# architector1324/micro-raytracer

Measured on AMD Instinct MI355X. Metric: Msamples/sec (res x spp), higher is better.
Workload: dtype f32

## Files before the change

micro_raytracer_amd/csrc/mrt_api.cpp:

```cpp
#include <hip/hip_runtime_api.h>
#include <dlfcn.h>
#include <stdarg.h>
#include <stddef.h>
#include <stdio.h>
#include <stdlib.h>
#include <string.h>

#include <chrono>
#include <memory>
#include <mutex>
#include <string>
#include <utility>
#include <vector>

#include "../../include/mrt.h"
#include "mrt_denoise.h"
#include "mrt_kernels.h"
#include "mrt_pack.h"
#include "mrt_trace.h"

using namespace mrt;

namespace {

// ... 269 lines not shown
struct Plan {
    bool in_lds = true;
    u32 block_threads = 256;
    bool small_plain_grid = false;
    size_t staged_bytes = 0;
};

void plan_launch(const mrt_render_desc *desc, const mrt_desc_ext *ext, Packed &pk, Plan &pl)
{
    const bool no_lds = getenv("MRT_SCENE_IN_L2") != nullptr;
    const char *force = getenv("MRT_BLOCK_THREADS");
    const bool mesh_walk = pk.n_tbvh_nodes != 0u && (pk.features & 3u) == 3u;
    u32 deep_cap = kWalkCapDefault;
    if (const char *fw = getenv("MRT_WALK_CAP")) { const int v = atoi(fw); if (v >= 4 && v <= (int)kWalkCapMax) deep_cap = (u32)v; }
    pk.P.walk_cap = mesh_walk ? kLeafQueue : 0u;
    auto lds_of = [&](u32 shape, u32 marker) { return pt_lds_bytes(pk.P, shape, true, (pk.features & 31u) | marker); };
    auto fits = [&](u32 shape, u32 marker) { return lds_of(shape, marker) <= kLdsLimit; };
    auto fits_any = [&](u32 marker) { return fits(256u, marker) || fits(512u, marker) || fits(1024u, marker); };
    auto waves = [&](u32 shape, u32 marker) {
        const size_t l = lds_of(shape, marker);
        return l > kLdsLimit ? (size_t)0 : (shape / 64u) * (kLdsLimit / (l ? l : 1));
    };
    constexpr u32 kWarm = 64u, kDeep = 64u | 128u;
    const bool has_warm = pk.P.lds_words_warm < pk.P.lds_words || mesh_walk;
    u32 cold = 0u;
    bool in_lds = !no_lds;
    if (in_lds) {
        const char *fc = getenv("MRT_COLD");
        const char *fd = getenv("MRT_DEEP_NODES");
        const bool warm_ok = has_warm && fits_any(kWarm) && !(fc && !atoi(fc));
        const bool all_ok = fits_any(0u) && !(fc && atoi(fc) && warm_ok);
        const bool bvh_no_mesh = (pk.features & 16u) != 0u && (pk.features & 2u) == 0u;
        if (fd && mesh_walk) cold = kDeep;
        else if (mesh_walk && warm_ok && fits(1024u, kWarm)) cold = kWarm;
        else if (bvh_no_mesh && warm_ok && !fc && waves(256u, 0u) < 16u && waves(256u, kWarm) >= 24u) cold = kWarm;
        else if (all_ok) cold = 0u;
        else if (warm_ok) cold = kWarm;
        else if (mesh_walk) cold = kDeep;
        else in_lds = false;
        if (cold == kDeep) {
            PackOpts po; po.tbvh_wide = true;
            Packed again; std::string err2;
            bool ok2 = pack_scene(desc, again, err2, po, ext) == MRT_OK && again.tbvh_wide;
            const size_t fixed = (size_t)ST_SLOTS * 1024u * sizeof(float) + (size_t)deep_cap * 1024u * sizeof(u32) + 1024u;
            const size_t front = ok2 ? (size_t)again.P.off_tbvh * 4 : 0;
            ok2 = ok2 && front + fixed < kLdsLimit;
            if (ok2) {
                const size_t room = (kLdsLimit - fixed - front) / (B4_WORDS * 4);
                size_t n = fd ? (size_t)strtoul(fd, nullptr, 10) : room;
                if (n > room) n = room;
                if (n > again.n_tbvh_nodes) n = again.n_tbvh_nodes;
                const u32 n_mesh = (again.P.off_node - again.P.off_mesh) / MESH_WORDS;
                ok2 = n >= n_mesh && n_mesh > 0u;
                if (ok2) {
                    const u32 keep = pk.features;
                    pk = again;
                    pk.features = keep;
                    pk.P.walk_cap = deep_cap;
                    pk.P.n_tbvh_hot = (u32)n;
                    pk.P.lds_words_hot = (pk.P.off_tbvh + (u32)n * B4_WORDS + 3u) & ~3u;
                }
            }
            if (!ok2) { cold = 0u; in_lds = false; }
        }
    }
    const size_t full_bytes = (size_t)pk.P.lds_words * 4;
    const size_t blob_bytes = in_lds ? (size_t)staged_words_for(pk.P, cold) * 4 : full_bytes;
    u32 want = 256u, marker = cold;
    pl.small_plain_grid = false;
    if (in_lds) {
        const size_t w256 = waves(256u, cold), w512 = waves(512u, cold), w1024 = waves(1024u, cold);
        if (w256 >= 16u) { want = 256u; pl.small_plain_grid = blob_bytes <= kSmallScene && !cold; }
        else if (w512 >= 16u) want = 512u;
        else if (w1024 >= 16u) want = 1024u;
        else if (w256 >= w512 && w256 >= 8u) want = 256u;
        else if (!cold && fits(1024u, 32u)) { want = 1024u; marker |= 32u; }
        else want = w1024 ? 1024u : (w512 ? 512u : 256u);
    }
    if (force && in_lds) {
        const u32 f = (u32)atoi(force);
        if ((f == 64u && !cold) || f == 256u || f == 512u || f == 1024u) { if (fits(f, cold)) { want = f; marker = cold; pl.small_plain_grid = false; } }
    }
    pk.features = (pk.features & (31u | F_VATTR | F_ENV)) | marker | (pk.all_ident ? (u32)F_IDENT : 0u);
    if (in_lds && marker == kWarm && mesh_walk && has_walk_area(pk.features)) {
        const size_t w0 = waves(want, marker);
        while (pk.P.walk_cap < kWalkCapMax) {
            ++pk.P.walk_cap;
            if (waves(want, marker) != w0) { --pk.P.walk_cap; break; }
        }
    }
    pl.in_lds = in_lds;
    pl.block_threads = want;
    pl.staged_bytes = blob_bytes;
}

}

static mrt_ctx *create_single(const mrt_render_desc *desc, const mrt_opts *opts, const mrt_desc_ext *ext)
{
    const u32 shard_count = opts->shard_count ? opts->shard_count : 1;
    if (opts->shard_index >= shard_count) { fail(MRT_ERR_ARG, "mrt_create: shard_index %u >= shard_count %u", opts->shard_index, shard_count); return nullptr; }

    std::unique_ptr<mrt_ctx> c(new mrt_ctx());
    std::string err;
    const int rc = pack_scene(desc, c->pk, err, PackOpts(), ext);
    if (rc != MRT_OK) { fail(rc, "mrt_create: %s", err.c_str()); return nullptr; }
    Plan plan;
    plan_launch(desc, ext, c->pk, plan);
    if (c->pk.tbvh_wide) {
        c->aov_pk.reset(new Packed());
        if (pack_scene(desc, *c->aov_pk, err, PackOpts(), ext) != MRT_OK) { fail(MRT_ERR_SCENE, "mrt_create: %s", err.c_str()); return nullptr; }
    }

    int ndev = 0;
    if (hipGetDeviceCount(&ndev) != hipSuccess || ndev <= 0) { fail(MRT_ERR_DEVICE, "mrt_create: no HIP device (this backend has no CPU path)"); return nullptr; }
    int dev = opts->device;
    if (dev < 0) { if (hipGetDevice(&dev) != hipSuccess) dev = 0; }
    if (dev >= ndev) { fail(MRT_ERR_ARG, "mrt_create: device %d of %d", dev, ndev); return nullptr; }
    c->device = dev;
    c->seed = opts->seed;
    c->shard_index = opts->shard_index; c->shard_count = shard_count;
    c->shard_rows = opts->shard_rows ? opts->shard_rows : 8;

    const u32 nh = c->pk.nh;
    for (u32 y = 0; y < nh; ++y) if ((y / c->shard_rows) % shard_count == c->shard_index) c->row_of.push_back(y);
    c->local_rows = (u32)c->row_of.size();

    auto bail = [&](int code, const char *what, hipError_t e) { fail(code, "mrt_create: %s: %s", what, hipGetErrorString(e)); return (mrt_ctx *)nullptr; };
    hipError_t e;
    if ((e = hipSetDevice(dev)) != hipSuccess) return bail(MRT_ERR_DEVICE, "hipSetDevice", e);
    if ((e = create(c->stream)) != hipSuccess) return bail(MRT_ERR_DEVICE, "hipStreamCreate", e);
    if ((e = create(c->ev0)) != hipSuccess) return bail(MRT_ERR_DEVICE, "hipEventCreate", e);
    if ((e = create(c->ev1)) != hipSuccess) return bail(MRT_ERR_DEVICE, "hipEventCreate", e);
    const size_t all_words = c->pk.blob.size();
    if ((e = c->blob.alloc(all_words ? all_words : 4)) != hipSuccess) return bail(MRT_ERR_DEVICE, "hipMalloc(scene)", e);
    if ((e = hipMemcpy(c->blob.p, c->pk.blob.data(), all_words * 4, hipMemcpyHostToDevice)) != hipSuccess) return bail(MRT_ERR_DEVICE, "hipMemcpy(scene)", e);
    {
        const u32 n_blocks = (nh + c->shard_rows - 1) / c->shard_rows;
        c->padded_rows = ((n_blocks + shard_count - 1) / shard_count) * c->shard_rows;
        if (shard_count == 1) c->padded_rows = nh;
    }
    if ((e = c->accum_own.alloc(plane_floats(c.get()))) != hipSuccess) return bail(MRT_ERR_DEVICE, "hipMalloc(accumulator)", e);
    c->d_accum = c->accum_own.p;
    if ((e = hipMemset(c->d_accum, 0, plane_floats(c.get()) * sizeof(float))) != hipSuccess) return bail(MRT_ERR_DEVICE, "hipMemset", e);
    if ((e = c->segments.alloc(8)) != hipSuccess) return bail(MRT_ERR_DEVICE, "hipMalloc", e);
    if ((e = hipMemset(c->segments.p, 0, 8 * sizeof(unsigned long long))) != hipSuccess) return bail(MRT_ERR_DEVICE, "hipMemset", e);

    c->scene_in_lds = plan.in_lds;
    c->small_plain_grid = plan.small_plain_grid;
    const u32 want = plan.block_threads;
    const size_t blob_bytes = plan.staged_bytes;
    c->block_threads = want;
    c->pk.P.tiles_x = want == 64u ? 1u : (want == 256u ? 2u : 4u);
    c->pk.P.tiles_y = want == 64u ? 1u : (want == 1024u ? 4u : 2u);
    if (c->scene_in_lds && (e = configure_pt_once(dev)) != hipSuccess) return bail(MRT_ERR_DEVICE, "hipFuncSetAttribute", e);

    c->P = c->pk.P;
    c->P.local_rows = c->local_rows; c->P.shard_index = c->shard_index; c->P.shard_count = c->shard_count; c->P.shard_rows = c->shard_rows;
    c->P.seed_lo = (u32)c->seed; c->P.seed_hi = (u32)(c->seed >> 32);
    c->P.blob = c->blob.p; c->P.accum = c->d_accum; c->P.segments = c->segments.p;
    c->P.tile_counter = reinterpret_cast<u32 *>(c->segments.p + 1);
    {
        int n_cu = 0;
        if (!hip_tolerated(hipDeviceGetAttribute(&n_cu, hipDeviceAttributeMultiprocessorCount, c->device)) || n_cu <= 0) n_cu = 256;
        const size_t lds = pt_lds_bytes(c->pk.P, c->block_threads, c->scene_in_lds, c->pk.features);
        size_t per_cu = 32u / (c->block_threads / 64u);
// ... 1029 lines not shown
```

micro_raytracer_amd/csrc/mrt_pack.cpp:

```cpp
#include "mrt_pack.h"

#include <math.h>
#include <stdio.h>
#include <string.h>

#include <algorithm>
#include <map>
#include <array>

namespace mrt {
namespace {

constexpr u32 kBvhMinInstances = 24;

struct H3 { float x, y, z; };
inline H3 h3(float x, float y, float z) { H3 r = {x, y, z}; return r; }
inline H3 hadd(H3 a, H3 b) { return h3(a.x + b.x, a.y + b.y, a.z + b.z); }
inline H3 hsub(H3 a, H3 b) { return h3(a.x - b.x, a.y - b.y, a.z - b.z); }
inline H3 hmuls(H3 a, float s) { return h3(a.x * s, a.y * s, a.z * s); }
inline H3 hneg(H3 a) { return h3(-a.x, -a.y, -a.z); }
inline H3 hhadam(H3 a, H3 b) { return h3(a.x * b.x, a.y * b.y, a.z * b.z); }
inline float hdot(H3 a, H3 b) { return a.x * b.x + a.y * b.y + a.z * b.z; }
inline H3 hcross(H3 a, H3 b) { return h3(a.y * b.z - a.z * b.y, a.z * b.x - a.x * b.z, a.x * b.y - a.y * b.x); }
inline float hmag(H3 a) { return sqrtf(a.x * a.x + a.y * a.y + a.z * a.z); }
// ... 622 lines not shown
            instx_tab.insert(instx_tab.end(), ix, ix + INSTX_WORDS);
            Bound bd;
            bd.ok = o.kind != MRT_KIND_PLANE;
            for (int a = 0; a < 3; ++a) bd.mn[a] = bd.mx[a] = 0.0f;
            if (bd.ok) {
                double lo[3] = {0, 0, 0}, hi[3] = {0, 0, 0}, rad = 0.0;
                if (o.kind == MRT_KIND_SPHERE) { rad = fabs((double)o.param[0]); for (int a = 0; a < 3; ++a) { lo[a] = -rad; hi[a] = rad; } }
                else if (o.kind == MRT_KIND_BOX) {
                    rad = 0.5 * sqrt((double)o.param[0] * o.param[0] + (double)o.param[1] * o.param[1] + (double)o.param[2] * o.param[2]);
                    for (int a = 0; a < 3; ++a) { hi[a] = 0.5 * fabs((double)o.param[a]); lo[a] = -hi[a]; }
                } else {
                    const float *vs = o.kind == MRT_KIND_TRIANGLE ? o.param : o.tris;
                    const size_t nv = o.kind == MRT_KIND_TRIANGLE ? 3 : (size_t)o.n_tris * 3;
                    for (int a = 0; a < 3; ++a) { lo[a] = INFINITY; hi[a] = -INFINITY; }
                    for (size_t v = 0; v < nv; ++v) {
                        const float *q = vs + v * 3;
                        const double m = sqrt((double)q[0] * q[0] + (double)q[1] * q[1] + (double)q[2] * q[2]);
                        if (!(m <= rad)) rad = m;
                        for (int a = 0; a < 3; ++a) { if (!(q[a] >= lo[a])) lo[a] = q[a]; if (!(q[a] <= hi[a])) hi[a] = q[a]; }
                    }
                    if (nv == 0) for (int a = 0; a < 3; ++a) lo[a] = hi[a] = 0.0;
                }
                const float *X = xf_tab.data() + (size_t)xf * XF_WORDS;
                const bool ident = bits(X[XF_IDENT]) != 0;
                bool ortho = true;
                if (!ident) {
                    double M[9];
                    for (int a = 0; a < 3; ++a) for (int b2 = 0; b2 < 3; ++b2) { double acc = 0; for (int k = 0; k < 3; ++k) acc += (double)X[XF_R + a * 3 + k] * X[XF_L + k * 3 + b2]; M[a * 3 + b2] = acc; }
                    for (int a = 0; a < 3 && ortho; ++a) for (int b2 = 0; b2 < 3; ++b2) { double acc = 0; for (int k = 0; k < 3; ++k) acc += M[a * 3 + k] * M[b2 * 3 + k]; if (!(fabs(acc - (a == b2 ? 1.0 : 0.0)) < 1e-4)) ortho = false; }
                    for (int a = 0; a < 3; ++a) { lo[a] = -rad; hi[a] = rad; }
                }
                const double pp[3] = {pos.x, pos.y, pos.z};
                bd.ok = ortho && rad < 1e6;
                for (int a = 0; a < 3 && bd.ok; ++a) {
                    const double slack = 1e-3 * fmax(fabs(lo[a]), fabs(hi[a])) + 1e-6;
                    bd.mn[a] = (float)(pp[a] + lo[a] - slack); bd.mx[a] = (float)(pp[a] + hi[a] + slack);
                    if (!(fabs(pp[a]) < 1e6) || !(bd.mn[a] <= bd.mx[a])) bd.ok = false;
                }
            }
            bounds.push_back(bd);
        }
        n_inst_total += o.n_inst;

        u32 mr[MAT_WORDS] = {0};
        mr[MAT_ALBEDO] = bits(o.mat.albedo[0]); mr[MAT_ALBEDO + 1] = bits(o.mat.albedo[1]); mr[MAT_ALBEDO + 2] = bits(o.mat.albedo[2]);
        mr[MAT_ROUGH] = bits(o.mat.rough); mr[MAT_METAL] = bits(o.mat.metal); mr[MAT_GLASS] = bits(o.mat.glass);
        mr[MAT_OPACITY] = bits(o.mat.opacity); mr[MAT_EMIT] = bits(o.mat.emit);
        for (int k = 0; k < 6; ++k) mr[MAT_MAP + k] = (u32)maps[k];
        if (tex_bilinear && any_map) {
            mr[MAT_FLAGS] = MATF_BILINEAR | (o.kind == MRT_KIND_SPHERE ? (u32)MATF_CLAMP_V : 0u);
            out.features |= 512u | 1024u;
        }
        mat_tab.insert(mat_tab.end(), mr, mr + MAT_WORDS);
    }
    if (xf_tab.empty()) { const float dflt[4] = {-0.0f, -0.0f, -1.0f, -0.0f}; xf_of(dflt); }

    P.n_rend = sc.n_renderer; P.n_inst = n_inst_total; P.n_light = sc.n_light;
    if (sc.n_light) out.features |= 8u;
    P.off_rend = B.align4(); B.w.insert(B.w.end(), rend_tab.begin(), rend_tab.end());
    std::vector<u32> lin_list, bvh_inst;
    std::vector<float> bvh_nodes;
    {
        std::vector<u32> elig;
        for (u32 i = 0; i < n_inst_total; ++i) (bounds[i].ok ? elig : lin_list).push_back(i);
        if (n_inst_total < kBvhMinInstances || elig.size() < kBvhMinInstances / 2) {
            lin_list.clear(); elig.clear();
        } else {
            std::vector<TriBox> ib(n_inst_total);
            for (u32 i : elig) for (int a = 0; a < 3; ++a) { ib[i].mn[a] = bounds[i].mn[a]; ib[i].mx[a] = bounds[i].mx[a]; ib[i].c[a] = 0.5f * bounds[i].mn[a] + 0.5f * bounds[i].mx[a]; }
            TbvhBuild build{ib, bvh_nodes, bvh_inst, MRT_IBVH_LEAF_MAX};
            build.make(elig, 0, elig.size());
            const u32 n_nodes = (u32)(bvh_nodes.size() / BVH_WORDS);
            for (u32 k = 0; k < n_nodes; ++k) { float *q = bvh_nodes.data() + (size_t)k * BVH_WORDS; if (bits(q[BVH_SKIP]) >= n_nodes) q[BVH_SKIP] = fbits(BVH_END); }
            out.features |= 16u;
        }
    }
    P.n_lin = (u32)lin_list.size(); P.n_bvh_nodes = (u32)(bvh_nodes.size() / BVH_WORDS);
    out.all_ident = n_inst_total > 0;
    const u32 xf0 = n_inst_total ? inst_tab[INST_TAG] >> TAG_XF_SHIFT : 0u;
    for (u32 i = 0; i < n_inst_total && out.all_ident; ++i) {
        const u32 tag = inst_tab[(size_t)i * INST_WORDS + INST_TAG];
        out.all_ident = (tag & TAG_IDENT) != 0u && memcmp(&xf_tab[tag >> TAG_XF_SHIFT], &xf_tab[xf0], XF_IDENT * sizeof(float)) == 0;
    }
    {
        float r_min = 3.0e38f;
        bool sphere = false;
        for (u32 i : bvh_inst) {
            if ((inst_tab[(size_t)i * INST_WORDS + INST_TAG] & TAG_KIND_MASK) != KIND_SPHERE) continue;
            sphere = true;
            for (int a = 0; a < 3; ++a) r_min = std::min(r_min, 0.5f * (bounds[i].mx[a] - bounds[i].mn[a]));
        }
        P.inst_k = 1e-4f;
        P.inst_ksq = !sphere ? 0.0f : (r_min > 1e-12f ? 4e-6f / r_min : 1e30f);
        P.inst_kpos = sphere ? 1e-5f : 2e-6f;
    }
    out.n_lin = P.n_lin; out.n_bvh_nodes = P.n_bvh_nodes;
    P.off_cam = B.align4(); for (int k = 0; k < 9; ++k) B.f(P.cam_L[k]); for (int k = 0; k < 9; ++k) B.f(P.cam_R[k]);
    P.off_lin = B.align4(); B.w.insert(B.w.end(), lin_list.begin(), lin_list.end());
    P.off_bvh = B.align4(); for (float v : bvh_nodes) B.f(v);
    P.off_bvhinst = B.align4(); B.w.insert(B.w.end(), bvh_inst.begin(), bvh_inst.end());
    P.off_inst = B.align4(); B.w.insert(B.w.end(), inst_tab.begin(), inst_tab.end());
    P.off_instx = B.align4(); B.w.insert(B.w.end(), instx_tab.begin(), instx_tab.end());
    P.off_xf = B.align4(); for (float v : xf_tab) B.f(v);
    P.off_mat = B.align4(); B.w.insert(B.w.end(), mat_tab.begin(), mat_tab.end());
    P.off_light = B.align4();
    for (u32 l = 0; l < sc.n_light; ++l) {
        const mrt_light &li = sc.light[l];
        if (li.kind > MRT_LIGHT_DIR) { err = "unknown light kind"; return MRT_ERR_SCENE; }
        B.u(li.kind);
        if (li.kind == MRT_LIGHT_POINT) B.f3(h3(li.v[0], li.v[1], li.v[2]));
        else B.f3(hnorm(hneg(hnorm(h3(li.v[0], li.v[1], li.v[2])))));
        B.f(li.pwr);
        B.f3(h3(li.color[0], li.color[1], li.color[2]));
    }
    P.off_tex = B.align4();
    const u32 tex_desc0 = (u32)B.w.size();
    B.w.resize(B.w.size() + (size_t)sc.n_textures * TEX_WORDS, 0);
    P.off_lut = B.align4();
    for (int k = 0; k < 256; ++k) B.f((float)k / 255.0f);
    if (opts.tbvh_wide) {
        struct Ref { u32 depth, mesh, local; };
        std::vector<Ref> order;
        std::vector<std::vector<u32>> newi(wide.size());
        for (size_t m = 0; m < wide.size(); ++m) { newi[m].resize(wide[m].size()); for (size_t k = 0; k < wide[m].size(); ++k) order.push_back({wide[m][k].depth, (u32)m, (u32)k}); }
        std::stable_sort(order.begin(), order.end(), [](const Ref &a, const Ref &b) { return a.depth < b.depth; });
        if (order.size() >= (1u << 24)) { err = "triangle BVHs too large"; return MRT_ERR_LIMIT; }
        for (size_t k = 0; k < order.size(); ++k) newi[order[k].mesh][order[k].local] = (u32)k;
        tbvh_tab.assign(order.size() * B4_WORDS, 0.0f);
        for (size_t k = 0; k < order.size(); ++k) {
            const Wide4 &w = wide[order[k].mesh][order[k].local];
            float *q = tbvh_tab.data() + k * B4_WORDS;
            for (int c = 0; c < 4; ++c) {
                q[B4_CX + c] = w.c[c][0]; q[B4_CY + c] = w.c[c][1]; q[B4_CZ + c] = w.c[c][2];
                q[B4_HX + c] = w.h[c][0]; q[B4_HY + c] = w.h[c][1]; q[B4_HZ + c] = w.h[c][2];
                u32 cw = w.child[c];
                if (cw & B4_INTERNAL) cw = B4_INTERNAL | newi[order[k].mesh][cw & ~B4_INTERNAL];
                q[B4_CHILD + c] = fbits(cw);
            }
        }
        for (size_t m = 0; m < wide.size(); ++m) mesh_tab[(size_t)wide_mesh[m] * MESH_WORDS + MESH_TBVH] = newi[m][0];
        out.tbvh_wide = true;
    }
    P.off_mesh = B.align4(); B.w.insert(B.w.end(), mesh_tab.begin(), mesh_tab.end());
    P.off_node = B.align4(); for (float v : node_tab) B.f(v);
    P.off_parent = B.align4(); B.w.insert(B.w.end(), parent_tab.begin(), parent_tab.end());
    P.off_tbvh = B.align4(); for (float v : tbvh_tab) B.f(v);
    P.lds_words_hot = B.align4();
    P.off_tri = B.align4(); for (float v : tri_tab) B.f(v);
    P.off_memb = B.align4(); B.w.insert(B.w.end(), memb_tab.begin(), memb_tab.end());
    P.off_membe = B.align4(); B.w.insert(B.w.end(), membe_tab.begin(), membe_tab.end());
    P.lds_words_warm = B.align4();
    for (u32 t = 0; t < sc.n_textures; ++t) {
        const mrt_texture &tx = sc.textures[t];
        u32 *desc = B.w.data() + tex_desc0 + (size_t)t * TEX_WORDS;
        desc[TEX_W] = tx.w; desc[TEX_H] = tx.h;
        if (!tx.dat) { desc[TEX_FMT] = TEXFMT_NONE; continue; }
        const size_t n = (size_t)tx.w * tx.h * 3;
        bool exact = true;
        for (size_t i = 0; i < n && exact; ++i) {
            const float v = tx.dat[i];
            const float kf = rintf(v * 255.0f);
            exact = kf >= 0.0f && kf <= 255.0f && bits(kf / 255.0f) == bits(v);
        }
        const u32 off = B.align4();
        desc = B.w.data() + tex_desc0 + (size_t)t * TEX_WORDS;
        if (exact) {
            desc[TEX_FMT] = TEXFMT_U8; desc[TEX_OFF] = off * 4u;
            std::vector<unsigned char> bytes(n);
            for (size_t i = 0; i < n; ++i) bytes[i] = (unsigned char)rintf(tx.dat[i] * 255.0f);
            const size_t words = (n + 3) / 4;
            const size_t at = B.w.size();
            B.w.resize(at + words, 0);
            memcpy(B.w.data() + at, bytes.data(), n);
            out.n_tex_u8++;
        } else {
            desc[TEX_FMT] = TEXFMT_F32; desc[TEX_OFF] = off;
            for (size_t i = 0; i < n; ++i) B.f(tx.dat[i]);
            out.n_tex_f32++;
        }
    }
    P.off_leaf = B.align4(); B.w.insert(B.w.end(), leaf_tab.begin(), leaf_tab.end());
    P.lds_words = P.off_leaf;
    if (!vattr_tab.empty()) {
        out.off_vattr = B.align4(); for (float v : vattr_tab) B.f(v);
        out.n_vattr_rows = (u32)(vattr_tab.size() / VATTR_WORDS);
// ... 39 lines not shown
```

micro_raytracer_amd/csrc/mrt_pack.h:

```cpp
#pragma once
#include <string>
#include <vector>

#include "../../include/mrt.h"
#include "mrt_scene.h"

namespace mrt {

struct Packed {
    Params P;
    std::vector<u32> blob;
    u32 nw = 0, nh = 0;
    u32 res_w = 0, res_h = 0;
    float gamma = 0, exp = 0;
    u32 features = 0;
    bool all_ident = false;
    bool tbvh_wide = false;
    u32 n_tex_u8 = 0, n_tex_f32 = 0, n_nodes = 0, n_leaf_ids = 0, n_tris = 0, n_xf = 0, n_bvh_nodes = 0, n_lin = 0, n_tbvh_nodes = 0;
    u32 off_vattr = 0, n_vattr_rows = 0;
};

struct PackOpts {
    bool tbvh_wide = false;
};

int pack_scene(const mrt_render_desc *desc, Packed &out, std::string &err, const PackOpts &opts = PackOpts(), const mrt_desc_ext *ext = nullptr);

struct OctreeFlat {
    std::vector<float> nodes;
    std::vector<u32> leaf_ids;
    u32 root = NO_NODE;
    bool empty_root = false;
};
void build_octree(const float *tris, u32 n_tris, OctreeFlat &out);

bool build_tbvh(const float *tris, u32 n_tris, std::vector<float> &nodes, std::vector<u32> &order);

struct ResampleTaps {
    std::vector<u32> left;
    std::vector<u32> count;
    std::vector<float> weight;
    u32 cap = 0;
};
void lanczos3_taps(u32 src, u32 dst, ResampleTaps &out);

}
```

micro_raytracer_amd/csrc/mrt_scene.h:

```cpp
#pragma once
#include <stddef.h>

#include "mrt_math.h"

namespace mrt {

constexpr u32 REND_WORDS = 16;
constexpr u32 INST_WORDS = 8;
constexpr u32 XF_WORDS = 20;
constexpr u32 MAT_WORDS = 16;
constexpr u32 LIGHT_WORDS = 8;
constexpr u32 TEX_WORDS = 4;
constexpr u32 MESH_WORDS = 12;
constexpr u32 TRI_WORDS = 9;
constexpr u32 NODE_WORDS = 8;

enum : u32 { REND_KIND = 0, REND_INST_OFF = 1, REND_INST_CNT = 2, REND_FLAGS = 3, REND_GEO = 4 };
enum : u32 { RF_HAS_MAPS = 1u, RF_HAS_UV = 2u, RF_HAS_VN = 4u };
enum : u32 { REND_VATTR = 15 };
constexpr u32 VATTR_WORDS = 16;
enum : u32 { VATTR_VN = 0, VATTR_UV = 9 };

enum : u32 { INST_POS = 0, INST_P3 = 3, INST_TAG = 4, INST_P5 = 5 };
enum : u32 { INSTX_REND = 0, INSTX_PLANE_NW = 1 };
constexpr u32 INSTX_WORDS = 4;
constexpr u32 TAG_KIND_MASK = 7u, TAG_IDENT = 8u, TAG_XF_SHIFT = 4u;

enum : u32 { XF_L = 0, XF_R = 9, XF_IDENT = 18 };

enum : u32 { MAT_ALBEDO = 0, MAT_ROUGH = 3, MAT_METAL = 4, MAT_GLASS = 5, MAT_OPACITY = 6, MAT_EMIT = 7, MAT_MAP = 8, MAT_FLAGS = 14 };
enum : u32 { MATF_BILINEAR = 1u, MATF_CLAMP_V = 2u };
enum : u32 { MAP_TEX = 0, MAP_ROUGH = 1, MAP_METAL = 2, MAP_GLASS = 3, MAP_OPACITY = 4, MAP_EMIT = 5 };

enum : u32 { LIGHT_KIND = 0, LIGHT_V = 1, LIGHT_PWR = 4, LIGHT_COLOR = 5 };

enum : u32 { TEX_W = 0, TEX_H = 1, TEX_OFF = 2, TEX_FMT = 3 };
enum : u32 { TEXFMT_NONE = 0, TEXFMT_F32 = 1, TEXFMT_U8 = 2 };

enum : u32 { ENV_W = 0, ENV_H = 1, ENV_OFF = 2, ENV_FMT = 3, ENV_MAP = 4, ENV_ROT = 5, ENV_PWR = 6, ENV_FLAGS = 7 };
enum : u32 { ENVF_BILINEAR = 1u };
constexpr u32 ENV_WORDS = 8;
enum : u32 { ENVMAP_SPHERE = 0, ENVMAP_LATLONG = 1 };

enum : u32 { MESH_TRI0 = 0, MESH_NTRI = 1, MESH_ROOT = 2, MESH_LEAF0 = 3, MESH_TBVH = 4, MESH_NIDS = 5, MESH_BC = 6, MESH_BH = 9 };
constexpr u32 NO_NODE = 0xffffffffu;

enum : u32 { NODE_HALF = 0, NODE_REL = 3, NODE_FIRST = 6, NODE_COUNT = 7 };

constexpr u32 B4_WORDS = 28;
constexpr u32 B4_INTERNAL = 0x80000000u;
constexpr u32 kWalkCapMin = 8u, kWalkCapMax = 16u, kWalkCapDefault = 16u;
enum : u32 { B4_CX = 0, B4_CY = 4, B4_CZ = 8, B4_HX = 12, B4_HY = 16, B4_HZ = 20, B4_CHILD = 24 };
constexpr u32 BVH_WORDS = 8;
constexpr u32 MEMB_SLOT_BITS = 22u, MEMB_SLOT_MASK = (1u << MEMB_SLOT_BITS) - 1u;
enum : u32 { BVH_C = 0, BVH_H = 3, BVH_SKIP = 6, BVH_LEAF = 7 };
constexpr u32 BVH_END = 0xffffffffu;

enum : u32 { KIND_SPHERE = 0, KIND_PLANE = 1, KIND_BOX = 2, KIND_TRIANGLE = 3, KIND_MESH = 4 };
enum : u32 { LK_POINT = 0, LK_DIR = 1 };

constexpr u32 kChunk = 16;

struct Params {
    u32 nw, nh;
    u32 local_rows, shard_index, shard_count, shard_rows;
    u32 n_samples, sample_base;
    u32 k_split;
    u32 to_planes;
    u32 seed_lo, seed_hi;
    u32 bounce;
    float q;
    float w, h, aspect;
    float inv2tan;
    float cam_pos[3];
    float aprt, foc;
    float cam_L[9], cam_R[9];
    u32 cam_ident;
    float sky[3];
    float sky_init[3];
    u32 n_rend, n_light, n_inst;
    u32 n_lin, n_bvh_nodes;
    float inst_ksq;
    float inst_k, inst_kpos;
    u32 off_lin, off_bvh, off_bvhinst;
    u32 off_cam;
    u32 off_rend, off_inst, off_instx, off_xf, off_mat, off_light, off_tex, off_lut, off_mesh, off_tri, off_node, off_leaf;
    u32 off_tbvh, off_memb, off_membe, off_parent;
    u32 n_tbvh_hot;
    u32 walk_cap;
    u32 blob_words;
    u32 lds_words;
    u32 lds_words_warm;
    u32 lds_words_hot;
    u32 tiles_x, tiles_y;
    u32 count_segments;
    const u32 *blob;
    float *accum;
    float *partial;
    unsigned long long partial_stride;
    unsigned long long *segments;
    u32 *tile_counter;
    u32 persist_grid;
    u32 off_env;
};
static_assert(sizeof(Params) % 8 == 0 && offsetof(Params, off_env) + 4 == sizeof(Params), "off_env fills the tail of Params");

struct TileList {
    const u32 *tiles;
    u32 n;
};

}
```

micro_raytracer_amd/csrc/mrt_trace.h:

```cpp
#pragma once
#include "mrt_scene.h"

namespace mrt {

enum : u32 {
    F_BOX = 1u,
    F_TRI = 2u,
    F_MAPS = 4u,
    F_LIGHTS = 8u,
    F_ALL = 15u,
    F_BVH = 16u,
    F_NOSTASH = 32u,
    F_COLD = 64u,
    F_DEEP = 128u,
    F_IDENT = 256u,
    F_ENV = 1024u,
    F_VATTR = 512u
};
constexpr u32 plain_feat(u32 feat) { return feat & ~(u32)F_IDENT; }
MRT_HD u32 staged_words_for(const Params &P, u32 feat) { return (feat & F_DEEP) ? P.lds_words_hot : ((feat & F_COLD) ? P.lds_words_warm : P.lds_words); }
constexpr bool has_walk_area(u32 feat) { return (feat & F_TRI) && (feat & F_BOX) && (feat & F_COLD); }
#ifndef MRT_UNIFORM_TAG
#define MRT_UNIFORM_TAG 1
#endif
#ifndef MRT_T0_FROM_KEY
#define MRT_T0_FROM_KEY 1
#endif
#ifndef MRT_NZFIN_PRODUCT
#define MRT_NZFIN_PRODUCT 1
#endif
#ifndef MRT_SHADOW_QUEUE
#define MRT_SHADOW_QUEUE 0
#endif
#ifndef MRT_LEAF_QUEUE
#define MRT_LEAF_QUEUE 8u
#endif
constexpr u32 kLeafQueue = MRT_LEAF_QUEUE;

#ifndef MRT_PROBE
#define MRT_PROBE(phase)
#endif
#ifndef MRT_COUNT
#define MRT_COUNT(counter)
#endif
#ifndef MRT_PROBE_INST
#define MRT_PROBE_INST(i)
#endif
#if defined(MRT_PHASE_TIMING) && defined(__HIP_DEVICE_COMPILE__)
#define MRT_TICK(slot) do { const unsigned long long now_ = __builtin_amdgcn_s_memtime(); phase_ticks[slot] += now_ - phase_last; phase_last = now_; } while (0)
#define MRT_TICK_DECL unsigned long long phase_ticks[4] = {0ull, 0ull, 0ull, 0ull}; unsigned long long phase_last = __builtin_amdgcn_s_memtime()
#define MRT_TICK_OUT(dst) do { for (int k_ = 0; k_ < 4; ++k_) (dst)[k_] = phase_ticks[k_]; } while (0)
#else
#define MRT_TICK(slot)
#define MRT_TICK_DECL
#define MRT_TICK_OUT(dst)
#endif
#ifndef MRT_PROBE_FALLBACK
#define MRT_PROBE_FALLBACK(ro, rd, dd)
#endif
#ifndef MRT_PROBE_ROUND
#define MRT_PROBE_ROUND(steps, tris, membs)
#endif
enum : u32 { CT_TRACE = 0, CT_LIN_TEST, CT_BVH_NODE, CT_BVH_TEST, CT_MESH_CALL, CT_MESH_ROOT_HIT, CT_TBVH_NODE, CT_TBVH_TRI, CT_TBVH_TRI_HIT, CT_MEMB_BOX, CT_TRACE_ANY, CT_WALK_OVERFLOW, CT_WALK_ROUND, CT_REF_TRI, CT_REF_BOX, CT_COUNT };
enum : u32 { PH_ITER = 0, PH_REGEN, PH_SPHERE_MATH, PH_PLANE_HIT, PH_SHADE, PH_NORMAL_NONPLANE, PH_SCATTER1, PH_SCATTER2, PH_REFRACT, PH_EMIT_END, PH_LIGHTS, PH_COUNT };

constexpr float kE = 0.0001f;
constexpr float kBig = 1.0f / 0.0001f;

struct V3 { float x, y, z; };
MRT_HD V3 v3(float x, float y, float z) { V3 r; r.x = x; r.y = y; r.z = z; return r; }
MRT_HD V3 add(V3 a, V3 b) { return v3(a.x + b.x, a.y + b.y, a.z + b.z); }
MRT_HD V3 sub(V3 a, V3 b) { return v3(a.x - b.x, a.y - b.y, a.z - b.z); }
MRT_HD float dot(V3 a, V3 b) { return a.x * b.x + a.y * b.y + a.z * b.z; }
MRT_HD V3 muls(V3 a, float s) { return v3(a.x * s, a.y * s, a.z * s); }
MRT_HD V3 neg(V3 a) { return v3(-a.x, -a.y, -a.z); }
MRT_HD V3 hadam(V3 a, V3 b) { return v3(a.x * b.x, a.y * b.y, a.z * b.z); }
MRT_HD V3 cross(V3 a, V3 b) { return v3(a.y * b.z - a.z * b.y, a.z * b.x - a.x * b.z, a.x * b.y - a.y * b.x); }
MRT_HD float mag(V3 a) { return sqrt_(a.x * a.x + a.y * a.y + a.z * a.z); }
MRT_HD V3 norm(V3 a) { return muls(a, recip_sqrt_(a.x * a.x + a.y * a.y + a.z * a.z)); }
MRT_HD V3 reflect(V3 d, V3 n) { return sub(d, muls(n, 2.0f * dot(d, n))); }
MRT_HD V3 m3mul(const float *m, V3 v)
{
    return v3(m[0] * v.x + m[1] * v.y + m[2] * v.z, m[3] * v.x + m[4] * v.y + m[5] * v.z, m[6] * v.x + m[7] * v.y + m[8] * v.z);
}
MRT_HD V3 ld3(const float *F, u32 i) { return v3(F[i], F[i + 1], F[i + 2]); }
struct alignas(16) F4 { float x, y, z, w; };
MRT_HD F4 ld4(const float *F, u32 i) { return *reinterpret_cast<const F4 *>(F + i); }
MRT_HD u32 ldu(const float *F, u32 i) { return f2u(F[i]); }

MRT_HD bool nzfin(float x)
{
#if defined(__HIP_DEVICE_COMPILE__)
    return __builtin_amdgcn_classf(x, 0x198);
#else
    const float a = fabs_(x);
    return a > 0.0f && a < kInf;
#endif
}
MRT_HD bool nzfin3(V3 v) { return nzfin(v.x) && nzfin(v.y) && nzfin(v.z); }
MRT_HD bool nzfin3_product(V3 v) { return MRT_NZFIN_PRODUCT ? nzfin((v.x * v.y) * v.z) : nzfin3(v); }
MRT_HD u32 mul24(u32 a, u32 b)
{
    return (a & 0xffffffu) * (b & 0xffffffu);
}
MRT_HD void sched_fence()
{
#if defined(__HIP_DEVICE_COMPILE__)
    __builtin_amdgcn_sched_barrier(0);
#endif
}
MRT_HD u32 opaque_v(u32 x)
{
#if defined(__HIP_DEVICE_COMPILE__)
    asm volatile("" : "+v"(x));
#endif
    return x;
}
MRT_HD u32 opaque_s(u32 x)
{
#if defined(__HIP_DEVICE_COMPILE__)
    asm volatile("" : "+s"(x));
#endif
    return x;
}
MRT_HD u32 lowest_bit(u32 x) { return (u32)__builtin_ctz(x | 0x80000000u); }

MRT_HD V3 xf_full(const float *X, V3 v) { return m3mul(X + XF_R, m3mul(X + XF_L, v)); }
MRT_HD V3 xf_vec(const float *X, bool ident, V3 v)
{
    if (ident && nzfin3_product(v)) return v;
    return xf_full(X, v);
}

MRT_HD V3 recip_patched(V3 d)
{
    V3 m;
#if defined(MRT_FAST_IEEE)
    if (wave_all(in_window(d.x) && in_window(d.y) && in_window(d.z))) {
        m = v3(div_core_(1.0f, d.x, rcp_refined_(d.x)), div_core_(1.0f, d.y, rcp_refined_(d.y)), div_core_(1.0f, d.z, rcp_refined_(d.z)));
        return m;
    }
#endif
    m = v3(1.0f / d.x, 1.0f / d.y, 1.0f / d.z);
    if (fabs_(m.x) == kInf) m.x = kBig;
    if (fabs_(m.y) == kInf) m.y = kBig;
    if (fabs_(m.z) == kInf) m.z = kBig;
    return m;
}

MRT_HD bool box_isect(V3 half, V3 ro, V3 m, V3 pos, float &t0, float &t1)
{
    const V3 n = hadam(sub(ro, pos), m);
    const V3 k = hadam(half, v3(fabs_(m.x), fabs_(m.y), fabs_(m.z)));
    const V3 a = sub(neg(n), k);
    const V3 b = add(neg(n), k);
    t0 = fmax_(fmax_(a.x, a.y), a.z);
    t1 = fmin_(fmin_(b.x, b.y), b.z);
    return !(t0 > t1 || t1 < 0.0f);
}

MRT_HD bool sphere_isect(float r2, V3 oo, V3 rd, float a, float &t0, float &t1)
{
    const float b = 2.0f * dot(oo, rd);
    const float c = dot(oo, oo) - r2;
    const float disc = b * b - 4.0f * a * c;
    if (disc < 0.0f) return false;
    if (b > 1e-20f && a > 0.0f && a < 1e18f && disc >= 0.0f) return false;
    MRT_PROBE(PH_SPHERE_MATH);
    const float sq = sqrt_(disc);
    float q0, q1;
    div2_(-b - sq, -b + sq, 2.0f * a, q0, q1);
// ... 689 lines not shown
template <bool ANY, u32 FEAT, bool UNIFORM = false>
MRT_HD bool isect_instance(const Scn &S, const RayPre &ray, u32 i, const F4 &ia, const F4 &ib, float &t0, float &t1, i32 &i0, i32 &i1, const float *X0 = nullptr)
{
    const float *F = S.U;
    const Params &P = *S.P;
    const V3 pos = v3(ia.x, ia.y, ia.z);
    const u32 tag = (UNIFORM && (FEAT & F_TRI) && MRT_UNIFORM_TAG) ? wave_uniform(f2u(ib.x)) : f2u(ib.x);
    const u32 kind = (UNIFORM && (FEAT & F_IDENT)) ? wave_uniform(tag & TAG_KIND_MASK) : (tag & TAG_KIND_MASK);
    const bool ident = (FEAT & F_IDENT) ? true : (tag & TAG_IDENT) != 0;
    const float *X = (FEAT & F_IDENT) ? X0 : F + P.off_xf + (tag >> TAG_XF_SHIFT);
    const V3 ro = add(pos, xf_vec(X, ident, sub(ray.o, pos)));
    const bool fast_d = (FEAT & F_IDENT) ? true : (ident && ray.d_ok);
    V3 rd = ray.d, m = ray.m;
    float dd = ray.dd;
    if (!fast_d) {
        rd = xf_full(X, ray.d);
        if constexpr (FEAT & F_BOX) m = recip_patched(rd);
        dd = dot(rd, rd);
    }
    t0 = 0.0f; t1 = 0.0f; i0 = -1; i1 = -1;
    if (kind == KIND_SPHERE) return sphere_isect(ia.w, sub(ro, pos), rd, dd, t0, t1);
    if (kind == KIND_PLANE) { const bool h = plane_isect(v3(ib.y, ib.z, ib.w), ia.w, ro, rd, t0); t1 = t0; return h; }
    if ((FEAT & F_BOX) && kind == KIND_BOX) return box_isect(v3(ia.w, ib.y, ib.z), ro, m, pos, t0, t1);
    if (FEAT & F_TRI) {
        const float *R = F + P.off_rend + ldu(F, P.off_instx + i * INSTX_WORDS + INSTX_REND) * REND_WORDS;
        if (kind == KIND_TRIANGLE) {
            const bool h = tri_isect(add(ld3(R, REND_GEO), pos), ld3(R, REND_GEO + 3), ld3(R, REND_GEO + 6), ro, rd, t0);
            t1 = t0;
            return h;
        }
        if ((FEAT & F_BOX) && kind == KIND_MESH) return mesh_isect<ANY, FEAT>(S, ldu(R, REND_GEO), ro, rd, dd, m, pos, t0, i0, t1, i1);
    }
    return false;
}

template <bool V> struct BoolTag { static constexpr bool value = V; };

template <bool ANY, u32 FEAT>
MRT_HD bool trace(const Scn &S, const RayPre &ray_, Hit &best)
{
    const float *F = S.U;
    const Params &P = *S.P;
    i32 best_key = 0x7fffffff;
    best.rend = -1; best.inst = 0; best.t0 = 0.0f; best.t1 = 0.0f; best.i0 = -1; best.i1 = -1;
    const float *I = F + P.off_inst;

    if (ANY) { MRT_COUNT(CT_TRACE_ANY); } else { MRT_COUNT(CT_TRACE); }
    const float *X0 = nullptr;
    RayPre ray_i = ray_;
    if constexpr (FEAT & F_IDENT) {
        X0 = F + P.off_xf + (ldu(I, INST_TAG) >> TAG_XF_SHIFT);
        if (!ray_.d_ok) {
            ray_i.d = xf_full(X0, ray_.d);
            if constexpr (FEAT & F_BOX) ray_i.m = recip_patched(ray_i.d);
            ray_i.dd = dot(ray_i.d, ray_i.d);
        }
    }
    const RayPre &ray = ray_i;
    auto consider = [&](u32 i, const F4 &ia, const F4 &ib, auto in_order, auto uniform) -> bool {
        float t0, t1;
        MRT_COUNT(CT_LIN_TEST);
        MRT_PROBE_INST(i);
        i32 i0, i1;
        if (!isect_instance<ANY, FEAT, decltype(uniform)::value>(S, ray, i, ia, ib, t0, t1, i0, i1, X0)) return false;
        if (ANY) return true;
        const i32 key = total_key(t0);
        const unsigned long long pair = ((unsigned long long)((u32)key ^ 0x80000000u) << 32) | i;
        const unsigned long long best_pair = ((unsigned long long)((u32)best_key ^ 0x80000000u) << 32) | (best.rend < 0 ? 0xffffffffu : best.inst);
        const bool better = decltype(in_order)::value ? key < best_key : pair < best_pair;
        if (better) {
            best_key = key;
            best.rend = 0; best.inst = i; best.t1 = t1; best.i0 = i0; best.i1 = i1;
            if constexpr ((FEAT & F_BVH) != 0 || !MRT_T0_FROM_KEY) best.t0 = t0;
        }
        return false;
    };
    using InOrder = BoolTag<(FEAT & F_BVH) == 0>;
    using AnyOrder = BoolTag<false>;
    using Shared = BoolTag<true>;
    using PerLane = BoolTag<false>;

    const bool bvh = (FEAT & F_BVH) != 0;
    const u32 n = bvh ? P.n_lin : P.n_inst;
    if (!bvh && !(FEAT & F_TRI) && n) {
        u32 j = 0;
        F4 a0 = ld4(I, 0), a1 = ld4(I, 4), b0 = a0, b1 = a1;
        for (;;) {
            if (j + 1u < n) { b0 = ld4(I, (j + 1u) * INST_WORDS); b1 = ld4(I, (j + 1u) * INST_WORDS + 4); }
            if (consider(j, a0, a1, InOrder(), Shared())) return true;
            if (++j >= n) break;
            if (j + 1u < n) { a0 = ld4(I, (j + 1u) * INST_WORDS); a1 = ld4(I, (j + 1u) * INST_WORDS + 4); }
            if (consider(j, b0, b1, InOrder(), Shared())) return true;
            if (++j >= n) break;
        }
    } else if (n) {
        const float *Lst = F + P.off_lin;
        u32 cur = bvh ? ldu(Lst, 0) : 0u;
        F4 qa = ld4(I, cur * INST_WORDS), qb = ld4(I, cur * INST_WORDS + 4);
        for (u32 j = 0; j < n; ++j) {
            const F4 ia = qa, ib = qb;
            const u32 i = cur;
            if (j + 1 < n) {
                cur = bvh ? ldu(Lst, j + 1) : j + 1;
                qa = ld4(I, cur * INST_WORDS); qb = ld4(I, cur * INST_WORDS + 4);
            }
            if (consider(i, ia, ib, InOrder(), Shared())) return true;
        }
    }

    if constexpr (bvh) {
        const bool cull = cull_ok(ray_.o, ray_.dd);
        const CullRay R = cull_ray(ray_.o, ray_.d);
        const float *N0 = F + P.off_bvh;
        u32 node = P.n_bvh_nodes ? 0u : BVH_END;
        V3 oinv, qm;
        float mg;
        {
            const F4 ra = ld4(N0, 0), rb = ld4(N0, 4);
            const V3 r = sub(v3(ra.x, ra.y, ra.z), R.o);
            const float ext = fmax_(fmax_(fabs_(r.x) + ra.w, fabs_(r.y) + rb.x), fabs_(r.z) + rb.y);
            const float obig = fmax_(fmax_(fabs_(ray_.o.x), fabs_(ray_.o.y)), fabs_(ray_.o.z));
            const float ksq = fmin_(P.inst_ksq * ext, 4e-3f) * MRT_MARGIN_SCALE;
            mg = fma_fast(P.inst_k * MRT_MARGIN_SCALE + ksq, ext, fma_fast(P.inst_kpos * MRT_MARGIN_SCALE, obig + obig + ext, 1e-6f * MRT_MARGIN_SCALE));
            oinv = hadam(R.o, R.inv);
            qm = muls(R.ainv, mg);
        }
        for (;;) {
            u32 leaf_a = 0u, leaf_b = 0u;
            bool walking = node != BVH_END;
            const float far = (!ANY && best.rend >= 0 && best.t0 >= 0.0f) ? best.t0 + 1e-3f * best.t0 + mg : kInf;
            while (walking) {
                const F4 na = ld4(N0, node * BVH_WORDS), nb = ld4(N0, node * BVH_WORDS + 4);
                MRT_COUNT(CT_BVH_NODE);
                const u32 skip = f2u(nb.z), leaf = f2u(nb.w);
                const float px = fma_fast(na.x, R.inv.x, -oinv.x), py = fma_fast(na.y, R.inv.y, -oinv.y), pz = fma_fast(na.z, R.inv.z, -oinv.z);
                const float qx = fma_fast(na.w, R.ainv.x, qm.x), qy = fma_fast(nb.x, R.ainv.y, qm.y), qz = fma_fast(nb.y, R.ainv.z, qm.z);
                const float tn = fmax_(fmax_(px - qx, py - qy), pz - qz);
                const float tf = fmin_(fmin_(px + qx, py + qy), pz + qz);
                bool hit_node = !(tn > tf || tf < 0.0f);
                if (!ANY) hit_node = hit_node && !(tn > far);
                hit_node = hit_node || !cull;
                const u32 cand = hit_node ? leaf : 0u;
                const bool have_a = leaf_a != 0u;
                leaf_b |= have_a ? cand : 0u;
                leaf_a |= have_a ? 0u : cand;
                node = (hit_node && leaf == 0u) ? node + 1u : skip;
                walking = node != BVH_END && leaf_b == 0u;
            }
            if (leaf_a == 0u) break;
            const u32 cnt_a = leaf_a >> 24, first_a = leaf_a & 0xffffffu, cnt_b = leaf_b >> 24, first_b = leaf_b & 0xffffffu;
            for (u32 k = 0; k < cnt_a + cnt_b; ++k) {
                const u32 i = ldu(F, P.off_bvhinst + (k < cnt_a ? first_a + k : first_b + (k - cnt_a)));
                if (consider(i, ld4(I, i * INST_WORDS), ld4(I, i * INST_WORDS + 4), AnyOrder(), PerLane())) return true;
            }
        }
    }
    if (best.rend < 0) return false;
    if constexpr ((FEAT & F_BVH) == 0 && MRT_T0_FROM_KEY) {
        const i32 k = best_key;
        best.t0 = u2f((u32)(k ^ (i32)(((u32)(k >> 31)) >> 1)));
    }
    best.rend = (i32)ldu(S.F, P.off_instx + best.inst * INSTX_WORDS + INSTX_REND);
    return true;
}

struct Obj {
    const float *R, *IX, *X;
// ... 469 lines not shown
```

Baseline: 9292.

## Add axis-aligned plane fast scan for identity-transform sphere/plane scenes

At pack time, scenes whose instances all share an identity transform and contain only spheres and axis-aligned planes get a compact per-instance table holding the plane axis code and signed distance. The trace loop gains a specialised linear scan for that case. It intersects axis-aligned planes with a single division along one axis instead of the general plane test, and keeps the sphere test. The aim is to cut arithmetic and instance-record loads in the primary intersection loop. The cost is extra code paths, a wave-uniform branch on the axis code, and float-exactness assumptions checked through bounds and wave_all guards. An env var can disable it.

```diff
diff --git a/micro_raytracer_amd/csrc/mrt_api.cpp b/micro_raytracer_amd/csrc/mrt_api.cpp
--- a/micro_raytracer_amd/csrc/mrt_api.cpp
+++ b/micro_raytracer_amd/csrc/mrt_api.cpp
@@ -375,6 +375,7 @@
         if ((f == 64u && !cold) || f == 256u || f == 512u || f == 1024u) { if (fits(f, cold)) { want = f; marker = cold; pl.small_plain_grid = false; } }
     }
     pk.features = (pk.features & (31u | F_VATTR | F_ENV)) | marker | (pk.all_ident ? (u32)F_IDENT : 0u);
+    if (const char *fa = getenv("MRT_AXIS_SCAN")) { if (!atoi(fa)) pk.P.axis_scan = 0u; }
     if (in_lds && marker == kWarm && mesh_walk && has_walk_area(pk.features)) {
         const size_t w0 = waves(want, marker);
         while (pk.P.walk_cap < kWalkCapMax) {
diff --git a/micro_raytracer_amd/csrc/mrt_pack.cpp b/micro_raytracer_amd/csrc/mrt_pack.cpp
--- a/micro_raytracer_amd/csrc/mrt_pack.cpp
+++ b/micro_raytracer_amd/csrc/mrt_pack.cpp
@@ -728,6 +728,26 @@
         const u32 tag = inst_tab[(size_t)i * INST_WORDS + INST_TAG];
         out.all_ident = (tag & TAG_IDENT) != 0u && memcmp(&xf_tab[tag >> TAG_XF_SHIFT], &xf_tab[xf0], XF_IDENT * sizeof(float)) == 0;
     }
+    std::vector<u32> axis_tab;
+    out.axis_scan = out.all_ident && out.features == 0u;
+    for (u32 i = 0; i < n_inst_total && out.axis_scan; ++i) {
+        const u32 *ir = &inst_tab[(size_t)i * INST_WORDS];
+        const u32 kind = ir[INST_TAG] & TAG_KIND_MASK;
+        auto bounded = [](u32 w) { return fabsf(fbits(w)) <= kAxisMax; };
+        u32 code = 0u, sd = 0u;
+        bool ok = bounded(ir[INST_POS]) && bounded(ir[INST_POS + 1]) && bounded(ir[INST_POS + 2]) && bounded(ir[INST_P3]);
+        if (kind == KIND_PLANE) {
+            u32 ones = 0u, zeros = 0u;
+            for (u32 k = 0; k < 3u; ++k) {
+                const u32 w = ir[INST_P5 + k], mag = w & 0x7fffffffu;
+                if (mag == 0x3f800000u) { ++ones; code = k + 1u; sd = ir[INST_P3] ^ (w & 0x80000000u); }
+                else if (mag == 0u) ++zeros;
+            }
+            ok = ok && ones == 1u && zeros == 2u;
+        } else if (kind != KIND_SPHERE) ok = false;
+        axis_tab.push_back(code); axis_tab.push_back(sd);
+        out.axis_scan = ok;
+    }
     {
         float r_min = 3.0e38f;
         bool sphere = false;
@@ -747,6 +767,8 @@
     P.off_bvhinst = B.align4(); B.w.insert(B.w.end(), bvh_inst.begin(), bvh_inst.end());
     P.off_inst = B.align4(); B.w.insert(B.w.end(), inst_tab.begin(), inst_tab.end());
     P.off_instx = B.align4(); B.w.insert(B.w.end(), instx_tab.begin(), instx_tab.end());
+    P.off_axis = 0u; P.axis_scan = out.axis_scan ? 1u : 0u;
+    if (out.axis_scan) { P.off_axis = B.align4(); B.w.insert(B.w.end(), axis_tab.begin(), axis_tab.end()); }
     P.off_xf = B.align4(); for (float v : xf_tab) B.f(v);
     P.off_mat = B.align4(); B.w.insert(B.w.end(), mat_tab.begin(), mat_tab.end());
     P.off_light = B.align4();
diff --git a/micro_raytracer_amd/csrc/mrt_pack.h b/micro_raytracer_amd/csrc/mrt_pack.h
--- a/micro_raytracer_amd/csrc/mrt_pack.h
+++ b/micro_raytracer_amd/csrc/mrt_pack.h
@@ -15,6 +15,7 @@
     float gamma = 0, exp = 0;
     u32 features = 0;
     bool all_ident = false;
+    bool axis_scan = false;
     bool tbvh_wide = false;
     u32 n_tex_u8 = 0, n_tex_f32 = 0, n_nodes = 0, n_leaf_ids = 0, n_tris = 0, n_xf = 0, n_bvh_nodes = 0, n_lin = 0, n_tbvh_nodes = 0;
     u32 off_vattr = 0, n_vattr_rows = 0;
diff --git a/micro_raytracer_amd/csrc/mrt_scene.h b/micro_raytracer_amd/csrc/mrt_scene.h
--- a/micro_raytracer_amd/csrc/mrt_scene.h
+++ b/micro_raytracer_amd/csrc/mrt_scene.h
@@ -24,6 +24,9 @@
 enum : u32 { INST_POS = 0, INST_P3 = 3, INST_TAG = 4, INST_P5 = 5 };
 enum : u32 { INSTX_REND = 0, INSTX_PLANE_NW = 1 };
 constexpr u32 INSTX_WORDS = 4;
+enum : u32 { AXIS_CODE = 0, AXIS_SD = 1 };
+constexpr u32 AXIS_WORDS = 2;
+constexpr float kAxisMax = 0x1p38f;
 constexpr u32 TAG_KIND_MASK = 7u, TAG_IDENT = 8u, TAG_XF_SHIFT = 4u;
 
 enum : u32 { XF_L = 0, XF_R = 9, XF_IDENT = 18 };
@@ -102,8 +105,10 @@
     u32 *tile_counter;
     u32 persist_grid;
     u32 off_env;
+    u32 off_axis;
+    u32 axis_scan;
 };
-static_assert(sizeof(Params) % 8 == 0 && offsetof(Params, off_env) + 4 == sizeof(Params), "off_env fills the tail of Params");
+static_assert(sizeof(Params) % 8 == 0 && offsetof(Params, axis_scan) + 4 == sizeof(Params), "Params has no tail padding");
 
 struct TileList {
     const u32 *tiles;
diff --git a/micro_raytracer_amd/csrc/mrt_trace.h b/micro_raytracer_amd/csrc/mrt_trace.h
--- a/micro_raytracer_amd/csrc/mrt_trace.h
+++ b/micro_raytracer_amd/csrc/mrt_trace.h
@@ -61,7 +61,7 @@
 #ifndef MRT_PROBE_ROUND
 #define MRT_PROBE_ROUND(steps, tris, membs)
 #endif
-enum : u32 { CT_TRACE = 0, CT_LIN_TEST, CT_BVH_NODE, CT_BVH_TEST, CT_MESH_CALL, CT_MESH_ROOT_HIT, CT_TBVH_NODE, CT_TBVH_TRI, CT_TBVH_TRI_HIT, CT_MEMB_BOX, CT_TRACE_ANY, CT_WALK_OVERFLOW, CT_WALK_ROUND, CT_REF_TRI, CT_REF_BOX, CT_COUNT };
+enum : u32 { CT_TRACE = 0, CT_LIN_TEST, CT_BVH_NODE, CT_BVH_TEST, CT_MESH_CALL, CT_MESH_ROOT_HIT, CT_TBVH_NODE, CT_TBVH_TRI, CT_TBVH_TRI_HIT, CT_MEMB_BOX, CT_TRACE_ANY, CT_WALK_OVERFLOW, CT_WALK_ROUND, CT_REF_TRI, CT_REF_BOX, CT_AXIS_SCAN, CT_COUNT };
 enum : u32 { PH_ITER = 0, PH_REGEN, PH_SPHERE_MATH, PH_PLANE_HIT, PH_SHADE, PH_NORMAL_NONPLANE, PH_SCATTER1, PH_SCATTER2, PH_REFRACT, PH_EMIT_END, PH_LIGHTS, PH_COUNT };
 
 constexpr float kE = 0.0001f;
@@ -87,6 +87,8 @@
 struct alignas(16) F4 { float x, y, z, w; };
 MRT_HD F4 ld4(const float *F, u32 i) { return *reinterpret_cast<const F4 *>(F + i); }
 MRT_HD u32 ldu(const float *F, u32 i) { return f2u(F[i]); }
+struct alignas(8) F2 { float x, y; };
+MRT_HD F2 ld2(const float *F, u32 i) { return *reinterpret_cast<const F2 *>(F + i); }
 
 MRT_HD bool nzfin(float x)
 {
@@ -942,7 +944,66 @@
 
     const bool bvh = (FEAT & F_BVH) != 0;
     const u32 n = bvh ? P.n_lin : P.n_inst;
-    if (!bvh && !(FEAT & F_TRI) && n) {
+    bool scanned = false;
+    if constexpr (!ANY && FEAT == F_IDENT && MRT_T0_FROM_KEY) {
+        const V3 o = ray_.o, d = ray_.d;
+        const bool tame = (int)in_window(d.x) & (int)in_window(d.y) & (int)in_window(d.z) & (int)(fabs_(o.x) <= kAxisMax) & (int)(fabs_(o.y) <= kAxisMax) &
+                          (int)(fabs_(o.z) <= kAxisMax);
+        if (P.axis_scan && n && wave_all(tame)) {
+            scanned = true;
+            MRT_COUNT(CT_AXIS_SCAN);
+            const float *A = F + P.off_axis;
+#if defined(MRT_FAST_IEEE)
+            const V3 r = v3(rcp_refined_(d.x), rcp_refined_(d.y), rcp_refined_(d.z));
+#else
+            const V3 r = v3(0.0f, 0.0f, 0.0f);
+#endif
+            auto plane = [&](u32 i, float ok, float dk, float rk, float pk, float sd) {
+                const float ro = pk + (ok - pk);
+                const float num = -(ro + sd);
+                float tt;
+#if defined(MRT_FAST_IEEE)
+                if (wave_all(fabs_(num) >= kWinLo)) tt = div_core_(num, dk, rk);
+                else
+#endif
+                    tt = num / dk;
+                (void)rk;
+                const i32 kb = (i32)f2u(tt);
+                if (kb > 0 && kb < best_key) { best_key = kb; best.inst = i; best.t1 = tt; }
+            };
+            auto test = [&](u32 i, const F4 &ia, const F2 &ax) {
+                MRT_COUNT(CT_LIN_TEST);
+                MRT_PROBE_INST(i);
+                const u32 code = wave_uniform(f2u(ax.x));
+                if (code == 1u) plane(i, o.x, d.x, r.x, ia.x, ax.y);
+                else if (code == 2u) plane(i, o.y, d.y, r.y, ia.y, ax.y);
+                else if (code == 3u) plane(i, o.z, d.z, r.z, ia.z, ax.y);
+                else {
+                    const V3 pos = v3(ia.x, ia.y, ia.z);
+                    const V3 ro = add(pos, xf_vec(X0, true, sub(o, pos)));
+                    float t0 = 0.0f, t1 = 0.0f;
+                    if (sphere_isect(ia.w, sub(ro, pos), d, ray_.dd, t0, t1)) {
+                        const i32 key = total_key(t0);
+                        if (key < best_key) { best_key = key; best.inst = i; best.t1 = t1; }
+                    }
+                }
+            };
+            u32 j = 0;
+            F4 a0 = ld4(I, 0), b0 = a0;
+            F2 c0 = ld2(A, 0), e0 = c0;
+            for (;;) {
+                if (j + 1u < n) { b0 = ld4(I, (j + 1u) * INST_WORDS); e0 = ld2(A, (j + 1u) * AXIS_WORDS); }
+                test(j, a0, c0);
+                if (++j >= n) break;
+                if (j + 1u < n) { a0 = ld4(I, (j + 1u) * INST_WORDS); c0 = ld2(A, (j + 1u) * AXIS_WORDS); }
+                test(j, b0, e0);
+                if (++j >= n) break;
+            }
+            best.rend = best_key != 0x7fffffff ? 0 : -1;
+        }
+    }
+    if (scanned) {
+    } else if (!bvh && !(FEAT & F_TRI) && n) {
         u32 j = 0;
         F4 a0 = ld4(I, 0), a1 = ld4(I, 4), b0 = a0, b1 = a1;
         for (;;) {
```

After: 9671 (median of 6 runs). +4.1%, better.
